# MGI-tech-bioinformatics/SuperPlus

Hardware: AMD Instinct MI355X
Metric: k-mers/s (DF createDict stage: trim + canonical k-mer count + solid filter + spectrum + adjacency) (higher is better)
Workload: dtype u64

## Files before the change

superplus_amd/csrc/dfk_kernels.h:

```cpp
#pragma once
#include <type_traits>
#include "dfk_device.h"
#include "dfk_fallback.h"
#include "dfk_scan_plan.h"

namespace dfk {

template <int K>
__global__ void __launch_bounds__(256)
k_trim(const uint8_t* __restrict__ pq, const uint64_t* __restrict__ pq_off, uint64_t pq_nbytes,
       const uint64_t* __restrict__ base_off, uint64_t packed_bytes, const uint32_t* __restrict__ read_len,
       uint64_t n_reads, uint32_t min_qual, uint32_t* __restrict__ good_len,
       unsigned long long* __restrict__ n_inst, unsigned int* __restrict__ bad,
       unsigned long long* __restrict__ sum_good)
{
    unsigned long long mine = 0, good = 0;
    bool any_bad = false;
    for (uint64_t r = (uint64_t)blockIdx.x * blockDim.x + threadIdx.x; r < n_reads; r += (uint64_t)gridDim.x * blockDim.x) {
        uint32_t gl = 0;
        uint64_t p = pq_off[r], end = pq_off[r + 1];
        uint32_t idx = 0, run = 0;
        const uint64_t b0 = base_off[r], b1 = base_off[r + 1];
        bool ok = p <= end && end <= pq_nbytes && b0 <= b1 && b1 <= packed_bytes && b1 - b0 >= ((uint64_t)read_len[r] + 3) / 4;
        if (!ok) end = p;
// ... 13 lines not shown
                uint64_t bit = 8 * (p + 1) + 9;
                const uint32_t fmask = (1u << nBits) - 1u;
                for (uint32_t left = nQs; left;) {
                    const uint64_t by = bit >> 3;
                    const uint32_t sh = (uint32_t)(bit & 7);
                    uint64_t w = 0;
                    if (by + 8 <= pq_nbytes) __builtin_memcpy(&w, pq + by, 8);
                    else for (uint32_t k = 0; k < 8 && by + k < pq_nbytes; ++k) w |= (uint64_t)pq[by + k] << (8 * k);
                    w >>= sh;
                    const uint32_t n = min(left, (64u - sh) / nBits);
                    for (uint32_t i = 0; i < n; ++i, w >>= nBits) {
                        const uint32_t q = minQ + ((uint32_t)w & fmask);
                        if (q < min_qual) run = 0;
                        else if (++run >= (uint32_t)K) gl = idx + 1;
                        ++idx;
                    }
                    bit += (uint64_t)n * nBits; left -= n;
                }
            }
            p += blk;
        }
        uint32_t rl = read_len[r];
        if (!ok || idx != rl) { any_bad = true; gl = 0; }
        if (gl > rl) gl = rl;
        good_len[r] = gl;
        good += gl;
        if (gl >= (uint32_t)K + 1) mine += gl - K + 1;
    }
    __shared__ unsigned long long sh[2][4];
    __shared__ unsigned int sh_bad;
    if (threadIdx.x == 0) sh_bad = 0;
    __syncthreads();
#pragma unroll
    for (int d = 32; d > 0; d >>= 1) { mine += __shfl_down(mine, d, 64); good += __shfl_down(good, d, 64); }
    if ((threadIdx.x & 63) == 0) { sh[0][threadIdx.x >> 6] = mine; sh[1][threadIdx.x >> 6] = good; }
    if (any_bad) atomicOr(&sh_bad, 1u);
    __syncthreads();
    if (threadIdx.x == 0) {
        unsigned long long a0 = sh[0][0] + sh[0][1] + sh[0][2] + sh[0][3], a1 = sh[1][0] + sh[1][1] + sh[1][2] + sh[1][3];
        if (a0) atomicAdd(n_inst, a0);
        if (a1) atomicAdd(sum_good, a1);
        if (sh_bad) atomicOr(bad, 1u);
    }
}

struct PartParams {
    uint32_t M;
    uint32_t W;
    uint32_t log2_nb;
    uint32_t log2_world;
    int64_t  read_id0;
    uint32_t sub_lo;
    uint32_t sub_n;
    uint32_t class_mask;
};

constexpr uint32_t SWEEP_CLASSES = 32;
__host__ __device__ inline uint32_t sweep_class_of(uint32_t local_bucket, uint32_t log2_local)
{ return log2_local > 5 ? local_bucket >> (log2_local - 5) : local_bucket; }
__host__ __device__ inline uint32_t sweep_class_mask(uint32_t sub_lo, uint32_t sub_n, uint32_t log2_local)
{
    if (sub_n == 0) return 0u;
    const uint32_t a = sweep_class_of(sub_lo, log2_local), b = sweep_class_of(sub_lo + sub_n - 1, log2_local);
    const uint32_t upto_b = b >= 31 ? 0xFFFFFFFFu : ((1u << (b + 1)) - 1u);
    return upto_b & ~((1u << a) - 1u);
}

constexpr uint32_t SUMMARY_OVERFLOW = 15;

__device__ __forceinline__ uint32_t pass_local(uint32_t bucket, const PartParams& pp)
{
    const uint32_t ls = pp.log2_nb - pp.log2_world;
    const uint32_t d = (bucket & ((1u << ls) - 1u)) - pp.sub_lo;
    return d < pp.sub_n ? (bucket >> ls) * pp.sub_n + d : 0xFFFFFFFFu;
}

__device__ __forceinline__ uint32_t bucket_of(uint32_t minhash, const PartParams& pp)
{
    const uint32_t b = (minhash * 0x9E3779B1u) >> (32 - pp.log2_nb);
    return ((b & ((1u << pp.log2_world) - 1u)) << (pp.log2_nb - pp.log2_world)) | (b >> pp.log2_world);
}
constexpr int PART_QCAP = 8;

template <int K>
__device__ __forceinline__ void emit_record(const uint32_t* __restrict__ words, uint64_t n_words, uint64_t bit0,
                                            uint32_t s0, uint32_t nk, uint32_t bucket, uint32_t gl, int32_t tag,
                                            uint64_t dst_index, uint4* __restrict__ records)
{
    const bool hp = s0 > 0;
    const bool hs = s0 + nk + (uint32_t)K <= gl;
    uint64_t bo = bit0 + 2ull * (hp ? s0 - 1 : 0);
    uint64_t wi = bo >> 5; uint32_t sh = (uint32_t)bo & 31u;
    uint32_t w[7];
#pragma unroll
    for (int i = 0; i < 7; ++i) w[i] = (wi + i < n_words) ? words[wi + i] : 0u;
    uint32_t o[6];
#pragma unroll
    for (int i = 0; i < 6; ++i) o[i] = alignbit(w[i + 1], w[i], sh);
    if (!hp) {
#pragma unroll
        for (int i = 5; i > 0; --i) o[i] = (o[i] << 2) | (o[i - 1] >> 30);
        o[0] <<= 2;
    }
    uint32_t nbits = 2u * (1u + nk + (uint32_t)K - 1u + (hs ? 1u : 0u));
#pragma unroll
    for (int i = 0; i < 6; ++i) {
        uint32_t lo = 32u * i;
        if (nbits <= lo) o[i] = 0;
        else if (nbits < lo + 32u) o[i] &= (1u << (nbits - lo)) - 1u;
    }
    uint4 a{rec_header(nk, hp, hs, bucket), (uint32_t)tag, o[0], o[1]};
    uint4 b{o[2], o[3], o[4], o[5]};
    records[2 * dst_index] = a;
    records[2 * dst_index + 1] = b;
}

__device__ __forceinline__ uint32_t class_bin(uint32_t bucket, const PartParams& pp)
{
    const uint32_t ls = pp.log2_nb - pp.log2_world;
    const uint32_t sub = bucket & ((1u << ls) - 1u);
    return (bucket >> ls) * PART_CLASSES + (ls > 6 ? sub >> (ls - 6) : sub);
}

template <int K, bool WRITE>
__device__ __forceinline__ void
partition_read(uint64_t r, uint32_t* smem, uint32_t* __restrict__ lh,
            const uint8_t* __restrict__ packed, uint64_t packed_bytes, const uint64_t* __restrict__ base_off,
            const uint32_t* __restrict__ good_len, const int32_t* __restrict__ bc, int64_t ign_bc_below,
            uint64_t n_reads, const PartParams& pp,
            unsigned long long* __restrict__ bucket_acc, unsigned long long* __restrict__ bucket_cur, uint64_t n_out,
            uint4* __restrict__ records, uint4* __restrict__ summaries, const uint32_t* __restrict__ read_list, uint64_t n_list,
            const uint64_t* __restrict__ slice_base, uint32_t* __restrict__ read_classes)
{
    auto place = [&](uint32_t b) -> uint64_t {
        if (!slice_base) { const uint64_t d = atomicAdd(&bucket_cur[b], 1ull); return d < n_out ? d : ~0ull; }
        const uint32_t owner = b / pp.sub_n;
        const uint64_t d = slice_base[owner] + atomicAdd(&bucket_cur[owner], 1ull);
        return d < slice_base[owner + 1] ? d : ~0ull;
    };
    uint32_t* arr = smem;
    uint32_t* queue = smem + pp.W * PART_THREADS;
    uint8_t* sidx = reinterpret_cast<uint8_t*>(smem + pp.W * PART_THREADS);
    uint32_t* ring = reinterpret_cast<uint32_t*>(sidx + pp.W * PART_THREADS);
    uint64_t sum_lo = 0, sum_hi = 0;
    const int tid = threadIdx.x;
    if (WRITE && read_list) { if (r >= n_list) return; r = read_list[r]; }
    const uint32_t M = pp.M, W = pp.W;
    const uint32_t gl = r < n_reads ? good_len[r] : 0;
    if (gl < (uint32_t)K + 1) {
        if (!WRITE && r < n_reads) { summaries[r] = uint4{0, 0, 0, 0}; if (read_classes) read_classes[r] = 0u; }
        return;
    }
    uint32_t Pi = 0, cur_rel = 0;
    uint32_t cmask = 0;
    const uint32_t log2_local = pp.log2_nb - pp.log2_world;

    const uint64_t byte0 = base_off[r];
    const uint32_t* words = reinterpret_cast<const uint32_t*>(packed);
    const uint64_t n_words = (packed_bytes + 3) >> 2;
    const uint64_t bit0 = byte0 * 8;
    int32_t tag = -1;
    if (bc && (int64_t)r + pp.read_id0 >= ign_bc_below) tag = bc[r];

    const uint32_t mmask = M == 16 ? 0xFFFFFFFFu : ((1u << (2 * M)) - 1u);
    const uint32_t rsh = 2 * (M - 1);
    uint32_t f = 0, rc = 0;
    uint32_t P = 0;
    uint32_t bi = 0;
    uint32_t cur_b = 0, cur_s0 = 0, cur_nk = 0;
    uint32_t qn = 0;

    uint64_t wi = bit0 >> 5;
    uint64_t filled_to = wi;
    auto fill = [&]() {
        uint32_t w[PART_RING];
#pragma unroll
        for (int k = 0; k < PART_RING; ++k) w[k] = filled_to + k < n_words ? words[filled_to + k] : 0u;
#pragma unroll
        for (int k = 0; k < PART_RING; ++k) ring[((filled_to + k) & (PART_RING - 1)) * PART_THREADS + tid] = w[k];
        filled_to += PART_RING;
    };
    uint32_t wbits, wnext = 0;
    if (!WRITE) { fill(); wbits = ring[(wi & (PART_RING - 1)) * PART_THREADS + tid]; }
    else { wbits = wi < n_words ? words[wi] : 0u; wnext = wi + 1 < n_words ? words[wi + 1] : 0u; }
    uint32_t wpos = (uint32_t)bit0 & 31u;
    uint32_t sfx_next = 0xFFFFFFFFu;

    auto close_run = [&]() {
        if (WRITE && cur_b == 0xFFFFFFFFu) return;
        if (!WRITE) {
            if (lh) { const uint32_t bin = class_bin(cur_b, pp); atomicAdd(&lh[bin], 1u); atomicAdd(&lh[(PART_CLASSES << pp.log2_world) + bin], cur_nk); }
            else atomicAdd(&bucket_acc[cur_b], (1ull << 32) | cur_nk);
            cmask |= 1u << sweep_class_of(cur_b & ((1u << log2_local) - 1u), log2_local);
            if (qn < (uint32_t)SUMMARY_RUNS) {
                const uint64_t fld = cur_nk | (cur_rel << 6);
                const uint32_t b = 8u + 12u * qn;
                if (b < 64u) { sum_lo |= fld << b; if (b > 52u) sum_hi |= fld >> (64u - b); }
// ... 365 lines not shown
    extern __shared__ uint32_t lh[];
    const uint32_t c = blockIdx.y;
    for (uint32_t i = threadIdx.x; i < n_sub; i += blockDim.x) lh[i] = 0;
    __syncthreads();
    const uint64_t n = min((uint64_t)fill[c], cap);
    const uint32_t* k = keys + c * cap;
    for (uint64_t t0 = (uint64_t)blockIdx.x * KEY_TILE; t0 < n; t0 += (uint64_t)gridDim.x * KEY_TILE) {
        const uint64_t t1 = min(n, t0 + KEY_TILE);
        uint4 v[KEY_VECS];
        key_tile_load(k, t0, t1, v);
        key_tile_each(t0, t1, v, [&](uint32_t key) { atomicAdd(&lh[key >> sh], 1u); });
    }
    __syncthreads();
    for (uint32_t i = threadIdx.x; i < n_sub; i += blockDim.x) if (lh[i]) atomicAdd(&sub_cnt[(uint64_t)c * n_sub + i], (unsigned long long)lh[i]);
}

__global__ void __launch_bounds__(1024)
k_keys_offsets(const unsigned long long* __restrict__ cnt, uint32_t n, unsigned long long* __restrict__ off, unsigned long long* __restrict__ cur)
{
    __shared__ unsigned long long part[1024];
    const uint32_t tid = threadIdx.x, per = (n + 1023) / 1024;
    const uint32_t lo = min(n, tid * per), hi = min(n, lo + per);
    unsigned long long s = 0;
    for (uint32_t i = lo; i < hi; ++i) s += cnt[i];
    part[tid] = s;
    __syncthreads();
    for (uint32_t d = 1; d < 1024; d <<= 1) {
        const unsigned long long v = tid >= d ? part[tid - d] : 0ull;
        __syncthreads();
        part[tid] += v;
        __syncthreads();
    }
    unsigned long long run = part[tid] - s;
    for (uint32_t i = lo; i < hi; ++i) { off[i] = run; cur[i] = run; run += cnt[i]; }
    if (tid == 1023) off[n] = part[1023];
}

__global__ void __launch_bounds__(256)
k_keys_partition(const uint32_t* __restrict__ keys, const unsigned long long* __restrict__ fill, uint64_t cap, uint32_t sh,
                 uint32_t n_sub, unsigned long long* __restrict__ cur, uint32_t* __restrict__ out)
{
    extern __shared__ unsigned long long lds64[];
    unsigned long long* base = lds64;
    uint32_t* lh = reinterpret_cast<uint32_t*>(lds64 + n_sub);
    const uint32_t c = blockIdx.y;
    const uint64_t n = min((uint64_t)fill[c], cap);
    const uint32_t* k = keys + c * cap;
    unsigned long long* cc = cur + (uint64_t)c * n_sub;
    for (uint64_t t0 = (uint64_t)blockIdx.x * KEY_TILE; t0 < n; t0 += (uint64_t)gridDim.x * KEY_TILE) {
        const uint64_t t1 = min(n, t0 + KEY_TILE);
        uint4 v[KEY_VECS];
        key_tile_load(k, t0, t1, v);
        for (uint32_t i = threadIdx.x; i < n_sub; i += blockDim.x) lh[i] = 0;
        __syncthreads();
        key_tile_each(t0, t1, v, [&](uint32_t key) { atomicAdd(&lh[key >> sh], 1u); });
        __syncthreads();
        for (uint32_t i = threadIdx.x; i < n_sub; i += blockDim.x) { if (lh[i]) base[i] = atomicAdd(&cc[i], (unsigned long long)lh[i]); lh[i] = 0; }
        __syncthreads();
        uint32_t sh2 = sh;
        asm volatile("" : "+s"(sh2));
        key_tile_each(t0, t1, v, [&](uint32_t key) { const uint32_t s = key >> sh2; out[base[s] + atomicAdd(&lh[s], 1u)] = key; });
        __syncthreads();
    }
}

__global__ void __launch_bounds__(1024)
k_keys_count(const uint32_t* __restrict__ part, const unsigned long long* __restrict__ off, uint32_t sb, unsigned long long* __restrict__ bucket_acc)
{
    __shared__ unsigned long long t[1u << KEY_SUB_BITS];
    const uint32_t s = blockIdx.x, nt = 1u << sb, m = nt - 1u;
    for (uint32_t i = threadIdx.x; i < nt; i += blockDim.x) t[i] = 0;
    __syncthreads();
    const uint64_t a = off[s], b = off[s + 1];
    for (uint64_t i = a + threadIdx.x; i < b; i += blockDim.x) {
        const uint32_t key = part[i];
        atomicAdd(&t[(key >> 6) & m], (1ull << 32) | (key & 63u));
    }
    __syncthreads();
    unsigned long long* dst = bucket_acc + ((uint64_t)s << sb);
    for (uint32_t i = threadIdx.x; i < nt; i += blockDim.x) if (t[i]) atomicAdd(&dst[i], t[i]);
}

constexpr int SLICE_READS = 16;
template <int K, bool EMIT, typename F>
__device__ __forceinline__ void for_each_run_in_pass(uint64_t r, const uint8_t* __restrict__ packed, uint64_t packed_bytes,
                                                     const uint64_t* __restrict__ base_off, const PartParams& pp,
                                                     const uint4* __restrict__ summaries, F&& f)
{
    const uint4 sm = summaries[r];
    const uint32_t n = sm.x & 15u;
    if (n == 0 || n == SUMMARY_OVERFLOW) return;
    const uint32_t* words = reinterpret_cast<const uint32_t*>(packed);
    const uint64_t n_words = (packed_bytes + 3) >> 2;
    const uint64_t bit0 = base_off[r] * 8;
    const uint32_t M = pp.M;
    const uint32_t mmask = M == 16 ? 0xFFFFFFFFu : ((1u << (2 * M)) - 1u);
    const uint64_t lo = (uint64_t)sm.x | ((uint64_t)sm.y << 32), hi = (uint64_t)sm.z | ((uint64_t)sm.w << 32);
    uint32_t s0 = 0;
#pragma unroll
    for (int i = 0; i < SUMMARY_RUNS; ++i) {
        if ((uint32_t)i < n) {
            constexpr int B0 = 8;
            const int b = B0 + 12 * i;
            const uint32_t fld = (uint32_t)(b + 12 <= 64 ? lo >> b : b >= 64 ? hi >> (b - 64) : (lo >> b) | (hi << (64 - b))) & 0xFFFu;
            const uint32_t nk = fld & 63u, rel = fld >> 6;
            const uint64_t bo = bit0 + 2ull * (s0 + rel);
            const uint64_t wi = bo >> 5;
            const uint32_t w0 = words[wi], w1 = wi + 1 < n_words ? words[wi + 1] : 0u;
            const uint32_t x = alignbit(w1, w0, (uint32_t)bo & 31u) & mmask;
            uint32_t y = __brev(x);
            y = ((y >> 1) & 0x55555555u) | ((y & 0x55555555u) << 1);
            const uint32_t fw = y >> (32 - 2 * M), rcv = ~x & mmask;
            const uint32_t bucket = bucket_of(mmer_hash(fw < rcv ? fw : rcv), pp);
            const uint32_t lb = pass_local(bucket, pp);
            if (lb != 0xFFFFFFFFu) f(s0, nk, lb, bucket >> (pp.log2_nb - pp.log2_world), bit0, (uint32_t)i + 1 == n);
            s0 += nk;
        }
    }
}

template <int K>
__global__ void __launch_bounds__(256)
k_scatter_slices(const uint8_t* __restrict__ packed, uint64_t packed_bytes, const uint64_t* __restrict__ base_off,
                 const uint32_t* __restrict__ good_len, const int32_t* __restrict__ bc, int64_t ign_bc_below,
                 uint64_t n_reads, PartParams pp, const uint4* __restrict__ summaries, const uint32_t* __restrict__ read_classes,
                 const uint64_t* __restrict__ slice_base,
                 unsigned long long* __restrict__ slice_fill,
                 uint4* __restrict__ records)
{
    __shared__ uint32_t cnt[256];
    __shared__ unsigned long long at[256];
    __shared__ uint16_t list[256 * SLICE_READS];
    __shared__ uint32_t n_list;
    const uint32_t world = 1u << pp.log2_world;
    const int lane = threadIdx.x & 63;
    const uint64_t r_block = (uint64_t)blockIdx.x * 256 * SLICE_READS;
    if (threadIdx.x < world) cnt[threadIdx.x] = 0;
    if (threadIdx.x == 0) n_list = 0;
    __syncthreads();
#pragma unroll
    for (int j = 0; j < SLICE_READS; ++j) {
        const uint32_t rel = 256u * j + threadIdx.x;
        const uint64_t r = r_block + rel;
        const bool hit = r < n_reads && (!read_classes || (read_classes[r] & pp.class_mask) != 0u);
        const unsigned long long mk = __ballot(hit);
        uint32_t w = 0;
        if (lane == 0 && mk) w = atomicAdd(&n_list, (uint32_t)__popcll(mk));
        w = __builtin_amdgcn_readfirstlane(w);
        if (hit) list[w + __popcll(mk & ((1ull << lane) - 1ull))] = (uint16_t)rel;
    }
    __syncthreads();
    const uint32_t n = n_list;
    for (uint32_t i = threadIdx.x; i < n; i += 256)
        for_each_run_in_pass<K, false>(r_block + list[i], packed, packed_bytes, base_off, pp, summaries,
                                       [&](uint32_t, uint32_t, uint32_t, uint32_t owner, uint64_t, bool) { atomicAdd(&cnt[owner], 1u); });
    __syncthreads();
    if (threadIdx.x < world) {
        const uint32_t m = cnt[threadIdx.x];
        at[threadIdx.x] = slice_base[threadIdx.x] + (m ? atomicAdd(&slice_fill[threadIdx.x], (unsigned long long)m) : 0ull);
        cnt[threadIdx.x] = 0;
    }
    __syncthreads();
    const uint32_t* words = reinterpret_cast<const uint32_t*>(packed);
    const uint64_t n_words = (packed_bytes + 3) >> 2;
    (void)good_len;
    for (uint32_t i = threadIdx.x; i < n; i += 256) {
        const uint64_t r = r_block + list[i];
        int32_t tag = -1;
        if (bc && (int64_t)r + pp.read_id0 >= ign_bc_below) tag = bc[r];
        for_each_run_in_pass<K, true>(r, packed, packed_bytes, base_off, pp, summaries,
            [&](uint32_t s0, uint32_t nk, uint32_t lb, uint32_t owner, uint64_t bit0, bool last) {
                const uint64_t dst = at[owner] + atomicAdd(&cnt[owner], 1u);
                if (dst < slice_base[owner + 1]) emit_record<K>(words, n_words, bit0, s0, nk, lb, last ? 0u : 0xFFFFFFFFu, tag, dst, records);
            });
    }
}

#ifndef DFK_SWEEP_READS
#define DFK_SWEEP_READS 8
#endif
template <int K> constexpr int sweep_reads() { return KTraits<K>::KW == 4 ? 2 : DFK_SWEEP_READS; }
template <int K>
__global__ void __launch_bounds__(256)
k_scatter_runs(const uint8_t* __restrict__ packed, uint64_t packed_bytes, const uint64_t* __restrict__ base_off,
               const uint32_t* __restrict__ good_len, const int32_t* __restrict__ bc, int64_t ign_bc_below,
               uint64_t n_reads, PartParams pp, const uint4* __restrict__ summaries, const uint32_t* __restrict__ read_classes,
               unsigned long long* __restrict__ bucket_cur, uint64_t n_out, uint4* __restrict__ records)
{
    constexpr int SWEEP_READS = sweep_reads<K>();
    __shared__ uint16_t list[256 * SWEEP_READS];
    __shared__ uint32_t n_list;
    (void)good_len;
    const int lane = threadIdx.x & 63;
    const uint64_t r_block = (uint64_t)blockIdx.x * 256 * SWEEP_READS;
    if (threadIdx.x == 0) n_list = 0;
    __syncthreads();
#pragma unroll
    for (int j = 0; j < SWEEP_READS; ++j) {
        const uint32_t rel = 256u * j + threadIdx.x;
        const uint64_t r = r_block + rel;
        const bool hit = r < n_reads && (read_classes[r] & pp.class_mask) != 0u;
        const unsigned long long mk = __ballot(hit);
        uint32_t at = 0;
        if (lane == 0 && mk) at = atomicAdd(&n_list, (uint32_t)__popcll(mk));
        at = __builtin_amdgcn_readfirstlane(at);
        if (hit) list[at + __popcll(mk & ((1ull << lane) - 1ull))] = (uint16_t)rel;
    }
    __syncthreads();
    const uint32_t n = n_list;
    const uint32_t* words = reinterpret_cast<const uint32_t*>(packed);
    const uint64_t n_words = (packed_bytes + 3) >> 2;
    for (uint32_t i = threadIdx.x; i < n; i += 256) {
        const uint64_t r = r_block + list[i];
        int32_t tag = -1;
        if (bc && (int64_t)r + pp.read_id0 >= ign_bc_below) tag = bc[r];
        for_each_run_in_pass<K, true>(r, packed, packed_bytes, base_off, pp, summaries,
            [&](uint32_t s0, uint32_t nk, uint32_t lb, uint32_t, uint64_t bit0, bool last) {
                const uint64_t dst = atomicAdd(&bucket_cur[lb], 1ull);
                if (dst < n_out) emit_record<K>(words, n_words, bit0, s0, nk, lb, last ? 0u : 0xFFFFFFFFu, tag, dst, records);
            });
    }
}



struct CountParams {
    uint32_t min_freq, min_bc;
    uint32_t n_items;
    uint32_t single;
    uint64_t seg_cap;
    uint32_t do_adj;
    uint32_t keep_pre;
};

struct CountGlobals {
    unsigned long long n_distinct;
    unsigned long long big_cursor;
    unsigned int next_item;
    unsigned int n_overflow;
    unsigned int solid_overflow;
    unsigned int n_split;
    unsigned long long n_boundary;
    unsigned long long part_cursor;
    unsigned int n_wg_idle;
    unsigned int pad_idle;
};

constexpr int COUNT_HIST_BINS = 256;
constexpr uint32_t COUNT_MAX_PROBE = 96;
constexpr uint32_t HIST_GLOBAL_BINS = 1u << 24;
constexpr uint32_t FLAG_SOLID = 0x80000000u;

template <int K> struct WaveStage {
    uint32_t rec[COUNT_CHUNK * 8 + 8];
    uint32_t starts[COUNT_CHUNK];
    uint32_t msk[64];
    uint32_t pc[64];
};

__device__ __forceinline__ uint32_t tld(const uint32_t* p)
{ return __hip_atomic_load(p, __ATOMIC_RELAXED, __HIP_MEMORY_SCOPE_AGENT); }
__device__ __forceinline__ void tst(uint32_t* p, uint32_t v)
{ __hip_atomic_store(p, v, __ATOMIC_RELAXED, __HIP_MEMORY_SCOPE_AGENT); }

struct Probe {
    uint32_t k0, k1, k2, k3, ctx, fp, step, slot;
    int32_t tag;
    bool active;
};

__device__ __forceinline__ Probe probe_begin(u128 c, uint32_t ctx, int32_t tag, uint32_t S, bool active)
{
    const uint32_t h = key_hash(c);
    return Probe{(uint32_t)c.lo, (uint32_t)(c.lo >> 32), (uint32_t)c.hi, (uint32_t)(c.hi >> 32), ctx, (h >> 24) | 1u,
                 ((h >> 11) | 1u) & (S - 1), h & (S - 1), tag, active};
}

#define DFK_COMPILER_FENCE() asm volatile("" ::: "memory")
#ifdef DFK_PHASE_TIMES
__device__ unsigned long long g_phase[16];
struct PhaseClock {
    unsigned long long t, acc[12];
    __device__ __forceinline__ void start() { t = __builtin_amdgcn_s_memtime(); for (int i = 0; i < 12; ++i) acc[i] = 0; }
    __device__ __forceinline__ void mark(int i) { const unsigned long long n = __builtin_amdgcn_s_memtime(); acc[i] += n - t; t = n; }
    __device__ __forceinline__ void flush(int lane) { if (lane == 0) for (int i = 0; i < 12; ++i) atomicAdd(&g_phase[i], acc[i]); }
};
#define PH(i) phase.mark(i)
#else
#define PH(i) do { } while (0)
#endif
__device__ unsigned int g_big_fail[4];

enum : uint32_t { PS_PROBING = 0, PS_FOUND = 1, PS_FAILED = 2, PS_IDLE = 3 };
constexpr uint32_t PROBE_COST = 1u << 12, PROBE_LIMIT = (COUNT_MAX_PROBE + 1) * PROBE_COST;

template <int KW, int NBC, bool LDS_TABLE>
__device__ __forceinline__ bool table_insert(uint32_t* __restrict__ keys, uint32_t* __restrict__ cnt,
                                             uint32_t* __restrict__ ctxs, uint32_t* __restrict__ bcw,
                                             uint32_t S, const Probe& A, uint32_t& n_claimed)
{
    uint32_t state = A.active ? PS_PROBING : PS_IDLE, slot = A.slot, seen = 0, cost = 0, waits = 0;
    while (__ballot(state == PS_PROBING) != 0ull) {
        if (state == PS_PROBING) {
            uint32_t e = 0, r0, r1, r2, r3 = A.k3;
            if (LDS_TABLE) {
                __hip_atomic_compare_exchange_strong(&cnt[slot], &e, CNT_LOCK, __ATOMIC_RELAXED, __ATOMIC_RELAXED,
                                                     __HIP_MEMORY_SCOPE_WORKGROUP);
                DFK_COMPILER_FENCE();
                r0 = tld(&keys[slot]); r1 = tld(&keys[S + slot]); r2 = tld(&keys[2 * S + slot]);
                if (KW == 4) r3 = tld(&keys[3 * S + slot]);
            } else {
                __hip_atomic_compare_exchange_strong(&cnt[slot], &e, CNT_LOCK, __ATOMIC_ACQUIRE, __ATOMIC_ACQUIRE,
                                                     __HIP_MEMORY_SCOPE_AGENT);
                r0 = tld(&keys[slot]); r1 = tld(&keys[S + slot]); r2 = tld(&keys[2 * S + slot]);
                if (KW == 4) r3 = tld(&keys[3 * S + slot]);
            }
            const bool won = e == 0u;
            if (won) {
                tst(&keys[slot], A.k0); tst(&keys[S + slot], A.k1); tst(&keys[2 * S + slot], A.k2);
                if (KW == 4) tst(&keys[3 * S + slot], A.k3);
                if (LDS_TABLE) {
                    DFK_COMPILER_FENCE();
                    __hip_atomic_store(&cnt[slot], A.fp << 24, __ATOMIC_RELAXED, __HIP_MEMORY_SCOPE_WORKGROUP);
                } else __hip_atomic_store(&cnt[slot], A.fp << 24, __ATOMIC_RELEASE, __HIP_MEMORY_SCOPE_AGENT);
            }
            const uint32_t locked = e == CNT_LOCK;
            const uint32_t match = ((e >> 24) == A.fp) & (r0 == A.k0) & (r1 == A.k1) & (r2 == A.k2) & (r3 == A.k3);
            const uint32_t fin = (uint32_t)won | match;
            n_claimed += (uint32_t)won;
            seen |= e & (0u - match);
            cost += PROBE_COST - (PROBE_COST - 1u) * locked;
            if (!LDS_TABLE) waits += locked;
            slot = (slot + (A.step & ((fin | locked) - 1u))) & (S - 1);
            state = fin | ((uint32_t)(cost >= PROBE_LIMIT) << 1);
        }
    }
    if (!LDS_TABLE && state == PS_FAILED && atomicCAS(&g_big_fail[0], 0u, 1u) == 0u) {
        g_big_fail[1] = (cost - waits) / PROBE_COST; g_big_fail[2] = waits; g_big_fail[3] = 31u - (uint32_t)__clz(S);
    }
    if (state == PS_FOUND) {
        if (LDS_TABLE) {
// ... 390 lines not shown
            PH(7);
        } else {
            for (uint32_t lo = 0; lo < S; lo += ADJ_TASKS / 8) {
                __syncthreads();
                if (tid == 0) tst(n_tasks, 0u);
                __syncthreads();
                for (uint32_t slot = lo + tid; slot < min(S, lo + ADJ_TASKS / 8); slot += nthreads) {
                    if (!(tld(&cnt[slot]) && (tld(&bcw[slot]) & FLAG_SOLID))) continue;
                    const uint32_t ctx = tld(&ctxs[slot]) & 0xFFu;
                    uint32_t pos = atomicAdd(n_tasks, __popc(ctx));
                    for (uint32_t bit = 0; bit < 8; ++bit) if (ctx & (1u << bit)) tasks[pos++] = slot | (bit << 28);
                }
                __syncthreads();
                const uint32_t n = __builtin_amdgcn_readfirstlane(tld(n_tasks));
                for (uint32_t t = tid; t < n; t += nthreads) resolve(tasks[t]);
            }
            sync();
        }
    }
    else sync();
    uint32_t boundary = 0;
    auto emit = [&](uint32_t slot, uint32_t c, uint32_t flags, unsigned long long idx) {
        const uint32_t count = c & CNT_MASK;
        const uint32_t cw = tld(&ctxs[slot]);
        const uint32_t pending = flags & 0xFFu & cw;
        boundary += pending != 0;
        if (idx < cp.seg_cap) {
            u128 v{(uint64_t)tld(&keys[slot]) | ((uint64_t)tld(&keys[S + slot]) << 32),
                   (uint64_t)tld(&keys[2 * S + slot]) | (KW == 4 ? ((uint64_t)tld(&keys[3 * S + slot]) << 32) : 0ull)};
            u128 kw = shl128(v, 128 - KTraits<K>::BITS);
            seg_out[2 * idx] = uint4{(uint32_t)kw.hi, (uint32_t)(kw.hi >> 32), (uint32_t)kw.lo, (uint32_t)(kw.lo >> 32)};
            seg_out[2 * idx + 1] = uint4{0xFFFFFFFFu, count | ((cw & 0xFFu) << 24), 0xFFFFFFFFu, pending | (cw & 0xFF00u)};
        } else atomicOr(seg_overflow, 1u);
        if (count < (uint32_t)COUNT_HIST_BINS) atomicAdd(&hist_lds[count], 1u);
        else atomicAdd(&hist_global[count], 1ull);
    };
    {
        const uint32_t ns = __builtin_amdgcn_readfirstlane(tld(n_solid));
        const uint32_t used = __builtin_amdgcn_readfirstlane(tld(&ctl[CTL_USED]));
        const unsigned long long cur = uniform64(tld(&ctl[CTL_OUT_LO]), tld(&ctl[CTL_OUT_HI]));
        const unsigned long long nxt = uniform64(tld(&ctl[CTL_NEXT_LO]), tld(&ctl[CTL_NEXT_HI]));
        for (uint32_t i = tid; i < ns; i += nthreads) {
            const uint32_t slot = solid_list[i];
            const uint32_t pos = used + i;
            emit(slot, tld(&cnt[slot]), tld(&bcw[slot]), pos < OUT_CHUNK ? cur + pos : nxt + (pos - OUT_CHUNK));
        }
        PH(8);
        __syncthreads();
        PH(9);
        if (tid == 0) {
            if (used + ns > OUT_CHUNK) { tst(&ctl[CTL_OUT_LO], (uint32_t)nxt); tst(&ctl[CTL_OUT_HI], (uint32_t)(nxt >> 32)); tst(&ctl[CTL_USED], used + ns - OUT_CHUNK); }
            else tst(&ctl[CTL_USED], used + ns);
            tst(n_solid, 0u);
        }
        uint4* z = reinterpret_cast<uint4*>(cnt);
        for (uint32_t i = tid; i < (3 + (NBC > 1 ? NBC - 1 : 0)) * S / 4; i += nthreads) z[i] = uint4{0, 0, 0, 0};
    }
    boundary = wave_sum(boundary);
    if (lane == 0 && boundary) atomicAdd(n_boundary, boundary);
    PH(10);
    return n_occ;
}


template <int K, int LOG2S, int NWAVES, int NBC, bool SUB>
__global__ void __launch_bounds__(NWAVES * 64)
k_count(const uint4* __restrict__ records, const ItemRange* __restrict__ items, const uint64_t* __restrict__ rec_base,
        CountParams cp, CountGlobals* __restrict__ g, uint4* __restrict__ out, WgOut* __restrict__ wg_out,
        unsigned long long* __restrict__ hist_global, ItemRange* __restrict__ overflow_items,
        const uint32_t* __restrict__ item_sub,
        unsigned int* __restrict__ resident)
{
    constexpr uint32_t S = 1u << LOG2S;
    constexpr int KW = KTraits<K>::KW;
    constexpr int NT = NWAVES * 64;
    extern __shared__ __align__(16) uint32_t smem[];
    uint32_t* keys = smem;
    uint32_t* cnt = keys + KW * S;
    uint32_t* ctxs = cnt + S;
    uint32_t* bcw = ctxs + S;
    constexpr uint32_t XW = NBC > 1 ? NBC - 1 : 0;
    uint32_t* hist = bcw + (1 + XW) * S;
    uint32_t* ctl = hist + COUNT_HIST_BINS;
    uint32_t* tasks = ctl + CTL_N;
    uint16_t* solid_list = reinterpret_cast<uint16_t*>(tasks + S / 2);
    WaveStage<K>* stages = reinterpret_cast<WaveStage<K>*>(tasks + S / 2 + S / 2);
    const int tid = threadIdx.x, lane = tid & 63, wave = tid >> 6;
    WaveStage<K>* st = stages + wave;
    uint4* seg_out = out;

    if (tid == 0 && resident) __hip_atomic_fetch_add(resident, 1u, __ATOMIC_RELAXED, __HIP_MEMORY_SCOPE_AGENT);
    for (int i = tid; i < COUNT_HIST_BINS; i += NT) hist[i] = 0;
    for (uint32_t i = tid; i < (3 + XW) * S; i += NT) cnt[i] = 0;
    if (tid == 0) {
        const WgOut w = wg_out[blockIdx.x];
        ctl[CTL_OUT_LO] = (uint32_t)w.chunk; ctl[CTL_OUT_HI] = (uint32_t)(w.chunk >> 32); ctl[CTL_USED] = w.used;
        ctl[CTL_NEXT_LO] = 0; ctl[CTL_NEXT_HI] = 0; ctl[CTL_DISTINCT] = 0; ctl[CTL_BOUNDARY] = 0;
        ctl[CTL_OVF] = 0; ctl[CTL_FILL] = 0; ctl[CTL_CHUNK] = 0; ctl[CTL_NTASK] = 0; ctl[CTL_NSOLID] = 0; ctl[CTL_SP] = 0;
        const uint32_t it0 = atomicAdd(&g->next_item, 1u);
        uint64_t b0 = 0, e0 = 0; ItemRange r0{0, 0}; uint32_t s0 = 0;
        if (it0 < cp.n_items) { r0 = items[it0]; b0 = rec_base[r0.b0]; e0 = rec_base[r0.b1]; if (SUB) s0 = item_sub[it0]; }
        ctl[CTL_ITEM] = it0; ctl[CTL_RB_LO] = (uint32_t)b0; ctl[CTL_RB_HI] = (uint32_t)(b0 >> 32);
        ctl[CTL_RE_LO] = (uint32_t)e0; ctl[CTL_RE_HI] = (uint32_t)(e0 >> 32);
        ctl[CTL_B0] = r0.b0; ctl[CTL_B1] = r0.b1; ctl[CTL_SUB] = s0;
    }
#ifdef DFK_PHASE_TIMES
    PhaseClock phase; phase.start();
#endif
    uint32_t items_done = 0;
    for (;;) {
        PH(0);
        __syncthreads();
        PH(1);
        const uint32_t item = __builtin_amdgcn_readfirstlane(ctl[CTL_ITEM]);
        if (item >= cp.n_items) break;
        ++items_done;
        const uint64_t rb = uniform64(ctl[CTL_RB_LO], ctl[CTL_RB_HI]);
        const uint64_t re = uniform64(ctl[CTL_RE_LO], ctl[CTL_RE_HI]);
        const uint32_t sub = __builtin_amdgcn_readfirstlane(ctl[CTL_SUB]);
        uint32_t nx = 0xFFFFFFFFu; uint64_t nb = 0, ne = 0; ItemRange nr{0, 0}; uint32_t nsub = 0;
        if (tid == 0 && ctl[CTL_SP] == 0) {
            nx = atomicAdd(&g->next_item, 1u);
            if (nx < cp.n_items) { nr = items[nx]; nb = rec_base[nr.b0]; ne = rec_base[nr.b1]; if (SUB) nsub = item_sub[nx]; }
        }
        const uint32_t n_rec = (uint32_t)(re - rb);
        const uint32_t share = (n_rec + NWAVES - 1) / NWAVES;
        const uint32_t wv = __builtin_amdgcn_readfirstlane((uint32_t)wave);
        const uint32_t w_lo = min(n_rec, wv * share), w_hi = min(n_rec, w_lo + share);
        if (!SUB && cp.single) {
            for (uint32_t at = w_lo; at < w_hi; at += 64) {
                if (__builtin_amdgcn_readfirstlane(tld(&ctl[CTL_OVF]))) break;
                const uint32_t r = at + (uint32_t)lane;
                uint4 a{0, 0, 0, 0}, b{0, 0, 0, 0};
                if (r < w_hi) { a = records[2 * (rb + r)]; b = records[2 * (rb + r) + 1]; }
                const InstRegs in{a.x, a.y, a.z, a.w, b.x, b.y, b.z, 0u};
                const Probe A = make_probe<K>(in, S, (a.x & 63u) != 0u);
                uint32_t claimed = 0;
                const bool ok = table_insert<KW, NBC, true>(keys, cnt, ctxs, bcw, S, A, claimed);
                claimed = wave_sum(claimed);
                if (lane == 0 && claimed) atomicAdd(&ctl[CTL_FILL], claimed);
                if (!ok) atomicOr(&ctl[CTL_OVF], 1u);
                if (lane == 0 && tld(&ctl[CTL_FILL]) > (S / 4) * 3) tst(&ctl[CTL_OVF], 1u);
            }
        } else
        for (uint32_t at = w_lo; at < w_hi; at += COUNT_CHUNK) {
            if (__builtin_amdgcn_readfirstlane(tld(&ctl[CTL_OVF]))) break;
            wave_count_chunk<K, NBC, true, SUB>(records, rb + at, rb + w_hi, st, lane, keys, cnt, ctxs, bcw, S,
                                             &ctl[CTL_FILL], &ctl[CTL_OVF], sub);
            if (lane == 0 && tld(&ctl[CTL_FILL]) > (S / 4) * 3) tst(&ctl[CTL_OVF], 1u);
        }
        PH(2);
        __syncthreads();
        PH(3);
        if (__builtin_amdgcn_readfirstlane(ctl[CTL_OVF])) {
            if (tid == 0) {
                const uint32_t b0 = ctl[CTL_B0], b1 = ctl[CTL_B1];
                uint32_t sp = ctl[CTL_SP];
                if (b1 - b0 > 1 && sp + 3 <= (uint32_t)CTL_STACK_CAP) {
                    if (nx < cp.n_items) { ctl[CTL_STACK + 3 * sp] = nr.b0; ctl[CTL_STACK + 3 * sp + 1] = nr.b1; ctl[CTL_STACK + 3 * sp + 2] = nsub; ++sp; nx = 0xFFFFFFFFu; }
                    const uint32_t mid = b0 + (b1 - b0) / 2;
                    ctl[CTL_STACK + 3 * sp] = mid; ctl[CTL_STACK + 3 * sp + 1] = b1; ctl[CTL_STACK + 3 * sp + 2] = 0u; ++sp;
                    ctl[CTL_STACK + 3 * sp] = b0; ctl[CTL_STACK + 3 * sp + 1] = mid; ctl[CTL_STACK + 3 * sp + 2] = 0u; ++sp;
                    ctl[CTL_SP] = sp;
                    atomicAdd(&g->n_split, 1u);
                } else overflow_items[atomicAdd(&g->n_overflow, 1u)] = ItemRange{b0, SUB ? (0x80000000u | ctl[CTL_SUB]) : b1};
            }
            for (uint32_t i = tid; i < (3 + XW) * S; i += NT) cnt[i] = 0;
            __syncthreads();
        } else {
            uint32_t occ = table_finish<K, NBC, S / 2>(keys, cnt, ctxs, bcw, S, cp, seg_out, ctl, &g->part_cursor,
                                                         &g->solid_overflow, hist, hist_global, tasks, &ctl[CTL_NTASK],
                                                         &ctl[CTL_BOUNDARY], solid_list, &ctl[CTL_NSOLID], tid, NT
#ifdef DFK_PHASE_TIMES
                                                         , phase
#endif
                                                         );
            occ = wave_sum(occ);
            if (lane == 0 && occ) atomicAdd(&ctl[CTL_DISTINCT], occ);
        }
        if (tid == 0) {
            const uint32_t sp = ctl[CTL_SP];
            uint32_t n0 = nr.b0, n1 = nr.b1;
            if (sp) {
                n0 = ctl[CTL_STACK + 3 * (sp - 1)]; n1 = ctl[CTL_STACK + 3 * (sp - 1) + 1]; nsub = ctl[CTL_STACK + 3 * (sp - 1) + 2];
                ctl[CTL_SP] = sp - 1;
                nx = 0; nb = rec_base[n0]; ne = rec_base[n1];
            }
            ctl[CTL_ITEM] = nx; ctl[CTL_RB_LO] = (uint32_t)nb; ctl[CTL_RB_HI] = (uint32_t)(nb >> 32);
            ctl[CTL_RE_LO] = (uint32_t)ne; ctl[CTL_RE_HI] = (uint32_t)(ne >> 32);
            ctl[CTL_B0] = n0; ctl[CTL_B1] = n1; ctl[CTL_SUB] = nsub;
            ctl[CTL_OVF] = 0; ctl[CTL_FILL] = 0; ctl[CTL_CHUNK] = 0; ctl[CTL_NTASK] = 0;
        }
    }
    __syncthreads();
#ifdef DFK_PHASE_TIMES
    PH(11); phase.flush(lane);
#endif
    for (int i = tid; i < COUNT_HIST_BINS; i += NT) if (hist[i]) atomicAdd(&hist_global[i], (unsigned long long)hist[i]);
    if (tid == 0) {
        wg_out[blockIdx.x] = WgOut{(unsigned long long)ctl[CTL_OUT_LO] | ((unsigned long long)ctl[CTL_OUT_HI] << 32), ctl[CTL_USED], 0u};
        if (ctl[CTL_DISTINCT]) atomicAdd(&g->n_distinct, (unsigned long long)ctl[CTL_DISTINCT]);
        if (ctl[CTL_BOUNDARY]) atomicAdd(&g->n_boundary, (unsigned long long)ctl[CTL_BOUNDARY]);
        if (!items_done) atomicAdd(&g->n_wg_idle, 1u);
    }
}

__global__ void __launch_bounds__(64)
k_gate(const unsigned int* __restrict__ ctr, unsigned int target, unsigned long long max_ticks, unsigned int* __restrict__ timed_out)
{
    if (threadIdx.x != 0) return;
    const unsigned long long t0 = wall_clock64();
    while ((int)(__hip_atomic_load(ctr, __ATOMIC_RELAXED, __HIP_MEMORY_SCOPE_AGENT) - target) < 0) {
        if (wall_clock64() - t0 > max_ticks) { __hip_atomic_fetch_add(timed_out, 1u, __ATOMIC_RELAXED, __HIP_MEMORY_SCOPE_AGENT); break; }
        __builtin_amdgcn_s_sleep(64);
    }
}

template <int K, int LOG2S, int NWAVES, int NBC>
constexpr size_t count_lds_bytes()
{
    return sizeof(uint32_t) * ((size_t)(KTraits<K>::KW + 3 + (NBC > 1 ? NBC - 1 : 0)) * (1u << LOG2S) + COUNT_HIST_BINS + CTL_N + (1u << LOG2S) / 2 + (1u << LOG2S) / 2) + sizeof(WaveStage<K>) * NWAVES;
}

template <int K, int NWAVES, int NBC>
__global__ void __launch_bounds__(NWAVES * 64)
k_big_insert(const uint4* __restrict__ records, const BigItem* __restrict__ items, const uint64_t* __restrict__ rec_base,
             const uint64_t* __restrict__ chunk_pre, uint32_t n_items, uint32_t* __restrict__ tab_pool,
             unsigned long long* __restrict__ ticket, uint32_t* __restrict__ failed)
{
    constexpr int KW = KTraits<K>::KW;
    __shared__ WaveStage<K> stages[NWAVES];
    __shared__ uint32_t fill, ovf;
    const int lane = threadIdx.x & 63, wave = threadIdx.x >> 6;
    if (threadIdx.x == 0) { fill = 0; ovf = 0; }
    __syncthreads();
    const uint64_t n_chunks = chunk_pre[n_items];
    for (uint32_t guard = 0; guard < 0x7FFFFFFFu; ++guard) {
        unsigned long long t0 = 0;
        if (lane == 0) t0 = atomicAdd(ticket, (unsigned long long)BIG_TICKET_CHUNKS);
        const uint64_t first = uniform64((uint64_t)t0);
        if (first >= n_chunks) break;
        for (int k = 0; k < BIG_TICKET_CHUNKS; ++k) {
            const uint64_t t = first + k;
            if (t >= n_chunks) break;
            const uint32_t it = big_find(chunk_pre, n_items, t);
            const BigItem I = items[it];
            const uint32_t S = 1u << I.log2s;
            uint32_t* keys = tab_pool + I.tab_off;
            uint32_t* cnt = keys + (size_t)KW * S;
            const uint64_t rb = rec_base[I.b0] + (t - chunk_pre[it]) * COUNT_CHUNK;
            wave_count_chunk<K, NBC, false>(records, rb, rec_base[I.b1], &stages[wave], lane, keys, cnt, cnt + S, cnt + 3 * (size_t)S, S, &fill, &ovf);
        }
    }
    __syncthreads();
    if (threadIdx.x == 0 && ovf) atomicOr(failed, 1u);
}

template <int K> struct BigView {
    uint32_t* keys; uint32_t* cnt; uint32_t* ctxs; uint32_t* wide; uint32_t* bcw; uint32_t S, slot;
    __device__ __forceinline__ uint32_t count() const { const uint32_t c = tld(&wide[slot]); return c < CNT_MASK ? c : CNT_MASK; }
};
template <int K>
__device__ __forceinline__ BigView<K> big_view(const BigItem* __restrict__ items, const uint64_t* __restrict__ slot_pre, uint32_t n_items,
                                               uint32_t* __restrict__ tab_pool, uint64_t x)
{
    const uint32_t it = big_find(slot_pre, n_items, x);
    const BigItem I = items[it];
    const uint32_t S = 1u << I.log2s;
    uint32_t* keys = tab_pool + I.tab_off;
    uint32_t* cnt = keys + (size_t)KTraits<K>::KW * S;
    return BigView<K>{keys, cnt, cnt + S, cnt + 2 * (size_t)S, cnt + 3 * (size_t)S, S, (uint32_t)(x - slot_pre[it])};
}

template <int K, int NBC>
__global__ void __launch_bounds__(256)
k_big_flags(const BigItem* __restrict__ items, const uint64_t* __restrict__ slot_pre, uint32_t n_items, uint32_t* __restrict__ tab_pool,
            CountParams cp, CountGlobals* __restrict__ g)
{
    const uint64_t total = slot_pre[n_items];
    uint32_t occ = 0;
    for (uint64_t x = (uint64_t)blockIdx.x * 256 + threadIdx.x; x < total; x += (uint64_t)gridDim.x * 256) {
        const BigView<K> v = big_view<K>(items, slot_pre, n_items, tab_pool, x);
        const uint32_t c = tld(&v.cnt[v.slot]);
        if (!c) continue;
        ++occ;
        const bool solid = v.count() >= cp.min_freq && bc_pass<(NBC > 0)>(NBC > 0 ? tld(&v.bcw[v.slot]) : 0u, cp.min_bc);
        if (solid && cp.do_adj && cp.keep_pre) { const uint32_t ctx = tld(&v.ctxs[v.slot]) & 0xFFu; tst(&v.ctxs[v.slot], ctx | (ctx << 8)); }
        tst(&v.bcw[v.slot], solid ? FLAG_SOLID : 0u);
    }
#pragma unroll
    for (int d = 32; d > 0; d >>= 1) occ += __shfl_down(occ, d, 64);
    if ((threadIdx.x & 63) == 0 && occ) atomicAdd(&g->n_distinct, (unsigned long long)occ);
}

template <int K>
__global__ void __launch_bounds__(256)
k_big_resolve(const BigItem* __restrict__ items, const uint64_t* __restrict__ slot_pre, uint32_t n_items, uint32_t* __restrict__ tab_pool)
{
    constexpr int KW = KTraits<K>::KW;
    const uint64_t total = slot_pre[n_items];
    const u128 m = KTraits<K>::mask();
    for (uint64_t x = (uint64_t)blockIdx.x * 256 + threadIdx.x; x < total; x += (uint64_t)gridDim.x * 256) {
        const BigView<K> v = big_view<K>(items, slot_pre, n_items, tab_pool, x);
        if (!tld(&v.cnt[v.slot]) || !(tld(&v.bcw[v.slot]) & FLAG_SOLID)) continue;
// ... 667 lines not shown
```

Before: 65.53 billion.

## Restructure scatter kernel into batched sweep with prefetch and alias count LDS lists

```diff
diff --git a/superplus_amd/csrc/dfk_kernels.h b/superplus_amd/csrc/dfk_kernels.h
--- a/superplus_amd/csrc/dfk_kernels.h
+++ b/superplus_amd/csrc/dfk_kernels.h
@@ -119,37 +119,50 @@
 }
 constexpr int PART_QCAP = 8;
 
+__device__ __forceinline__ void record_window_load(const uint32_t* __restrict__ words, uint64_t n_words, uint64_t bit0,
+                                                   uint32_t s0, uint32_t (&w)[7])
+{
+    const uint64_t wi = (bit0 + 2ull * (s0 > 0 ? s0 - 1 : 0)) >> 5;
+#pragma unroll
+    for (int i = 0; i < 7; ++i) w[i] = (wi + i < n_words) ? words[wi + i] : 0u;
+}
+
+template <int K>
+__device__ __forceinline__ void record_write(const uint32_t (&w)[7], uint64_t bit0, uint32_t s0, uint32_t nk, uint32_t bucket,
+                                             uint32_t gl, int32_t tag, uint64_t dst_index, uint4* __restrict__ records)
+{
+    const bool hp = s0 > 0;
+    const bool hs = s0 + nk + (uint32_t)K <= gl;
+    const uint32_t sh = (uint32_t)(bit0 + 2ull * (hp ? s0 - 1 : 0)) & 31u;
+    uint32_t o[6];
+#pragma unroll
+    for (int i = 0; i < 6; ++i) o[i] = alignbit(w[i + 1], w[i], sh);
+    if (!hp) {
+#pragma unroll
+        for (int i = 5; i > 0; --i) o[i] = (o[i] << 2) | (o[i - 1] >> 30);
+        o[0] <<= 2;
+    }
+    uint32_t nbits = 2u * (1u + nk + (uint32_t)K - 1u + (hs ? 1u : 0u));
+#pragma unroll
+    for (int i = 0; i < 6; ++i) {
+        uint32_t lo = 32u * i;
+        if (nbits <= lo) o[i] = 0;
+        else if (nbits < lo + 32u) o[i] &= (1u << (nbits - lo)) - 1u;
+    }
+    uint4 a{rec_header(nk, hp, hs, bucket), (uint32_t)tag, o[0], o[1]};
+    uint4 b{o[2], o[3], o[4], o[5]};
+    records[2 * dst_index] = a;
+    records[2 * dst_index + 1] = b;
+}
+
 template <int K>
 __device__ __forceinline__ void emit_record(const uint32_t* __restrict__ words, uint64_t n_words, uint64_t bit0,
                                             uint32_t s0, uint32_t nk, uint32_t bucket, uint32_t gl, int32_t tag,
                                             uint64_t dst_index, uint4* __restrict__ records)
 {
-    const bool hp = s0 > 0;
-    const bool hs = s0 + nk + (uint32_t)K <= gl;
-    uint64_t bo = bit0 + 2ull * (hp ? s0 - 1 : 0);
-    uint64_t wi = bo >> 5; uint32_t sh = (uint32_t)bo & 31u;
     uint32_t w[7];
-#pragma unroll
-    for (int i = 0; i < 7; ++i) w[i] = (wi + i < n_words) ? words[wi + i] : 0u;
-    uint32_t o[6];
-#pragma unroll
-    for (int i = 0; i < 6; ++i) o[i] = alignbit(w[i + 1], w[i], sh);
-    if (!hp) {
-#pragma unroll
-        for (int i = 5; i > 0; --i) o[i] = (o[i] << 2) | (o[i - 1] >> 30);
-        o[0] <<= 2;
-    }
-    uint32_t nbits = 2u * (1u + nk + (uint32_t)K - 1u + (hs ? 1u : 0u));
-#pragma unroll
-    for (int i = 0; i < 6; ++i) {
-        uint32_t lo = 32u * i;
-        if (nbits <= lo) o[i] = 0;
-        else if (nbits < lo + 32u) o[i] &= (1u << (nbits - lo)) - 1u;
-    }
-    uint4 a{rec_header(nk, hp, hs, bucket), (uint32_t)tag, o[0], o[1]};
-    uint4 b{o[2], o[3], o[4], o[5]};
-    records[2 * dst_index] = a;
-    records[2 * dst_index + 1] = b;
+    record_window_load(words, n_words, bit0, s0, w);
+    record_write<K>(w, bit0, s0, nk, bucket, gl, tag, dst_index, records);
 }
 
 __device__ __forceinline__ uint32_t class_bin(uint32_t bucket, const PartParams& pp)
@@ -681,6 +694,11 @@
 }
 
 constexpr int SLICE_READS = 16;
+__device__ __forceinline__ uint32_t summary_field(uint64_t lo, uint64_t hi, int i)
+{
+    const int b = 8 + 12 * i;
+    return (uint32_t)(b + 12 <= 64 ? lo >> b : b >= 64 ? hi >> (b - 64) : (lo >> b) | (hi << (64 - b))) & 0xFFFu;
+}
 template <int K, bool EMIT, typename F>
 __device__ __forceinline__ void for_each_run_in_pass(uint64_t r, const uint8_t* __restrict__ packed, uint64_t packed_bytes,
                                                      const uint64_t* __restrict__ base_off, const PartParams& pp,
@@ -699,9 +717,7 @@
 #pragma unroll
     for (int i = 0; i < SUMMARY_RUNS; ++i) {
         if ((uint32_t)i < n) {
-            constexpr int B0 = 8;
-            const int b = B0 + 12 * i;
-            const uint32_t fld = (uint32_t)(b + 12 <= 64 ? lo >> b : b >= 64 ? hi >> (b - 64) : (lo >> b) | (hi << (64 - b))) & 0xFFFu;
+            const uint32_t fld = summary_field(lo, hi, i);
             const uint32_t nk = fld & 63u, rel = fld >> 6;
             const uint64_t bo = bit0 + 2ull * (s0 + rel);
             const uint64_t wi = bo >> 5;
@@ -775,12 +791,96 @@
     }
 }
 
+constexpr int SWEEP_HITS = 2;
+constexpr uint32_t SWEEP_NONE = 0xFFFFFFFFu;
+struct SweepRead {
+    uint4 sm; uint64_t byte0;
+    __device__ __forceinline__ uint32_t n() const { const uint32_t c = sm.x & 15u; return c == SUMMARY_OVERFLOW ? 0u : c; }
+    __device__ __forceinline__ uint32_t sub() const { return ((uint32_t)byte0 & 3u) * 8u; }
+    __device__ __forceinline__ const uint32_t* rw(const uint32_t* __restrict__ words) const { return words + (byte0 >> 2); }
+};
+struct __attribute__((aligned(4))) SweepPair { uint32_t a, b; };
+struct SweepHits { uint32_t lb[SWEEP_HITS], runs; };
+
+__device__ __forceinline__ SweepRead sweep_read(uint64_t r, const uint64_t* __restrict__ base_off, const uint4* __restrict__ summaries)
+{
+    return SweepRead{summaries[r], base_off[r]};
+}
+
+constexpr int SWEEP_BATCH = SUMMARY_RUNS / 2;
+static_assert(2 * SWEEP_BATCH == SUMMARY_RUNS, "two batches cover a summary");
+
+template <int I0>
+__device__ __forceinline__ void sweep_min_words(const SweepRead& R, uint32_t n, const uint32_t* __restrict__ words, uint32_t s0,
+                                                uint32_t (&w)[SWEEP_BATCH][2])
+{
+    const uint64_t lo = (uint64_t)R.sm.x | ((uint64_t)R.sm.y << 32), hi = (uint64_t)R.sm.z | ((uint64_t)R.sm.w << 32);
+    const uint32_t* rw = R.rw(words);
+    const uint32_t sub = R.sub();
+#pragma unroll
+    for (int i = I0; i < I0 + SWEEP_BATCH; ++i) {
+        if ((uint32_t)i < n) {
+            const uint32_t fld = summary_field(lo, hi, i);
+            const SweepPair v = *reinterpret_cast<const SweepPair*>(rw + ((sub + 2u * (s0 + (fld >> 6))) >> 5));
+            w[i - I0][0] = v.a; w[i - I0][1] = v.b;
+            s0 += fld & 63u;
+        }
+    }
+}
+
+template <int I0>
+__device__ __forceinline__ void sweep_pick(const SweepRead& R, uint32_t n, const uint32_t (&w)[SWEEP_BATCH][2], const PartParams& pp,
+                                           uint32_t& s0, uint32_t& found, SweepHits& H)
+{
+    const uint64_t lo = (uint64_t)R.sm.x | ((uint64_t)R.sm.y << 32), hi = (uint64_t)R.sm.z | ((uint64_t)R.sm.w << 32);
+    const uint32_t M = pp.M;
+    const uint32_t mmask = M == 16 ? 0xFFFFFFFFu : ((1u << (2 * M)) - 1u);
+    const uint32_t sub = R.sub();
+#pragma unroll
+    for (int i = I0; i < I0 + SWEEP_BATCH; ++i) {
+        if ((uint32_t)i < n) {
+            const uint32_t fld = summary_field(lo, hi, i);
+            const uint32_t sh = (sub + 2u * (s0 + (fld >> 6))) & 31u;
+            const uint32_t x = alignbit(w[i - I0][1], w[i - I0][0], sh) & mmask;
+            uint32_t y = __brev(x);
+            y = ((y >> 1) & 0x55555555u) | ((y & 0x55555555u) << 1);
+            const uint32_t fw = y >> (32 - 2 * M), rcv = ~x & mmask;
+            const uint32_t lb = pass_local(bucket_of(mmer_hash(fw < rcv ? fw : rcv), pp), pp);
+            if (lb != SWEEP_NONE) {
+#pragma unroll
+                for (int g = 0; g < SWEEP_HITS; ++g) if (found == (uint32_t)g) { H.lb[g] = lb; H.runs |= (uint32_t)i << (4 * g); }
+                ++found;
+            }
+            s0 += fld & 63u;
+        }
+    }
+}
+
+__device__ __forceinline__ void sweep_window_load(const SweepRead& R, const uint32_t* __restrict__ words, uint32_t s0, uint32_t (&w)[7])
+{
+    const uint32_t* p = R.rw(words) + ((R.sub() + 2u * (s0 > 0 ? s0 - 1 : 0)) >> 5);
+#pragma unroll
+    for (int i = 0; i < 7; ++i) w[i] = p[i];
+}
+
+__device__ __forceinline__ void sweep_run(const SweepRead& R, uint32_t run, uint32_t& s0, uint32_t& nk)
+{
+    const uint64_t lo = (uint64_t)R.sm.x | ((uint64_t)R.sm.y << 32), hi = (uint64_t)R.sm.z | ((uint64_t)R.sm.w << 32);
+    s0 = 0; nk = 0;
+#pragma unroll
+    for (int i = 0; i < SUMMARY_RUNS; ++i) {
+        const uint32_t k = summary_field(lo, hi, i) & 63u;
+        if ((uint32_t)i < run) s0 += k;
+        if ((uint32_t)i == run) nk = k;
+    }
+}
+
 #ifndef DFK_SWEEP_READS
 #define DFK_SWEEP_READS 8
 #endif
 template <int K> constexpr int sweep_reads() { return KTraits<K>::KW == 4 ? 2 : DFK_SWEEP_READS; }
 template <int K>
-__global__ void __launch_bounds__(256)
+__global__ void __launch_bounds__(256, 8)
 k_scatter_runs(const uint8_t* __restrict__ packed, uint64_t packed_bytes, const uint64_t* __restrict__ base_off,
                const uint32_t* __restrict__ good_len, const int32_t* __restrict__ bc, int64_t ign_bc_below,
                uint64_t n_reads, PartParams pp, const uint4* __restrict__ summaries, const uint32_t* __restrict__ read_classes,
@@ -809,15 +909,73 @@
     const uint32_t n = n_list;
     const uint32_t* words = reinterpret_cast<const uint32_t*>(packed);
     const uint64_t n_words = (packed_bytes + 3) >> 2;
-    for (uint32_t i = threadIdx.x; i < n; i += 256) {
-        const uint64_t r = r_block + list[i];
+    const uint64_t r_end = r_block + 256ull * SWEEP_READS < n_reads ? r_block + 256ull * SWEEP_READS : n_reads;
+    if (base_off[r_end] + 32 > packed_bytes) {
+        for (uint32_t i = threadIdx.x; i < n; i += 256) {
+            const uint64_t r = r_block + list[i];
+            int32_t tag = -1;
+            if (bc && (int64_t)r + pp.read_id0 >= ign_bc_below) tag = bc[r];
+            for_each_run_in_pass<K, true>(r, packed, packed_bytes, base_off, pp, summaries,
+                [&](uint32_t s0, uint32_t nk, uint32_t lb, uint32_t, uint64_t bit0, bool last) {
+                    const uint64_t dst = atomicAdd(&bucket_cur[lb], 1ull);
+                    if (dst < n_out) emit_record<K>(words, n_words, bit0, s0, nk, lb, last ? 0u : 0xFFFFFFFFu, tag, dst, records);
+                });
+        }
+        return;
+    }
+    uint32_t i = threadIdx.x;
+    SweepRead R{};
+    if (i < n) R = sweep_read(r_block + list[i], base_off, summaries);
+    while (i < n) {
+        const uint32_t n_runs = R.n();
+        SweepHits H;
+#pragma unroll
+        for (int g = 0; g < SWEEP_HITS; ++g) H.lb[g] = SWEEP_NONE;
+        H.runs = 0u;
+        uint32_t before = 0, found = 0;
+        uint32_t w[SWEEP_BATCH][2];
+        sweep_min_words<0>(R, n_runs, words, before, w);
+        const SweepRead N = sweep_read(r_block + list[i + 256 < n ? i + 256 : i], base_off, summaries);
+        sweep_pick<0>(R, n_runs, w, pp, before, found, H);
+        if (__ballot(n_runs > (uint32_t)SWEEP_BATCH) != 0ull) {
+            sweep_min_words<SWEEP_BATCH>(R, n_runs, words, before, w);
+            sweep_pick<SWEEP_BATCH>(R, n_runs, w, pp, before, found, H);
+        }
+        uint32_t meta[SWEEP_HITS];
+#pragma unroll
+        for (int g = 0; g < SWEEP_HITS; ++g) {
+            const uint32_t run = (H.runs >> (4 * g)) & 15u;
+            uint32_t s0, nk;
+            sweep_run(R, run, s0, nk);
+            meta[g] = s0 | (nk << 16) | (run + 1u == n_runs ? 1u << 22 : 0u);
+        }
+        if (found > (uint32_t)SWEEP_HITS) meta[0] |= 1u << 23;
+        unsigned long long d[SWEEP_HITS];
+#pragma unroll
+        for (int g = 0; g < SWEEP_HITS; ++g) { d[g] = ~0ull; if (H.lb[g] != SWEEP_NONE) d[g] = atomicAdd(&bucket_cur[H.lb[g]], 1ull); }
         int32_t tag = -1;
-        if (bc && (int64_t)r + pp.read_id0 >= ign_bc_below) tag = bc[r];
-        for_each_run_in_pass<K, true>(r, packed, packed_bytes, base_off, pp, summaries,
-            [&](uint32_t s0, uint32_t nk, uint32_t lb, uint32_t, uint64_t bit0, bool last) {
-                const uint64_t dst = atomicAdd(&bucket_cur[lb], 1ull);
-                if (dst < n_out) emit_record<K>(words, n_words, bit0, s0, nk, lb, last ? 0u : 0xFFFFFFFFu, tag, dst, records);
-            });
+        if (H.lb[0] != SWEEP_NONE) {
+            const uint64_t r = r_block + list[i];
+            if (bc && (int64_t)r + pp.read_id0 >= ign_bc_below) tag = bc[r];
+        }
+#pragma unroll
+        for (int g = 0; g < SWEEP_HITS; ++g) {
+            if (H.lb[g] == SWEEP_NONE) continue;
+            uint32_t pw[7];
+            sweep_window_load(R, words, meta[g] & 0xFFFFu, pw);
+            if (d[g] < n_out) record_write<K>(pw, R.sub(), meta[g] & 0xFFFFu, (meta[g] >> 16) & 63u, H.lb[g], ((meta[g] >> 22) & 1u) ? 0u : 0xFFFFFFFFu, tag, d[g], records);
+        }
+        if (meta[0] >> 23) {
+            uint32_t seen = 0;
+            for_each_run_in_pass<K, true>(r_block + list[i], packed, packed_bytes, base_off, pp, summaries,
+                [&](uint32_t s0, uint32_t nk, uint32_t lb, uint32_t, uint64_t bit0, bool last) {
+                    if (seen++ < (uint32_t)SWEEP_HITS) return;
+                    const uint64_t dst = atomicAdd(&bucket_cur[lb], 1ull);
+                    if (dst < n_out) emit_record<K>(words, n_words, bit0, s0, nk, lb, last ? 0u : 0xFFFFFFFFu, tag, dst, records);
+                });
+        }
+        R = N;
+        i += 256;
     }
 }
 
@@ -856,6 +1014,7 @@
     uint32_t msk[64];
     uint32_t pc[64];
 };
+template <int LOG2S> constexpr size_t count_finish_bytes() { return sizeof(uint32_t) * ((1u << LOG2S) / 2) + sizeof(uint16_t) * (1u << LOG2S); }
 
 __device__ __forceinline__ uint32_t tld(const uint32_t* p)
 { return __hip_atomic_load(p, __ATOMIC_RELAXED, __HIP_MEMORY_SCOPE_AGENT); }
@@ -1412,9 +1571,11 @@
     constexpr uint32_t XW = NBC > 1 ? NBC - 1 : 0;
     uint32_t* hist = bcw + (1 + XW) * S;
     uint32_t* ctl = hist + COUNT_HIST_BINS;
+    static_assert((CTL_N % 4) == 0 && (S / 2) % 4 == 0 && sizeof(WaveStage<K>) % 16 == 0, "the staging areas and the lists stay 16-byte aligned");
+    static_assert(count_finish_bytes<LOG2S>() <= sizeof(WaveStage<K>) * NWAVES, "the finish lists fit the staging areas of this many waves");
     uint32_t* tasks = ctl + CTL_N;
     uint16_t* solid_list = reinterpret_cast<uint16_t*>(tasks + S / 2);
-    WaveStage<K>* stages = reinterpret_cast<WaveStage<K>*>(tasks + S / 2 + S / 2);
+    WaveStage<K>* stages = reinterpret_cast<WaveStage<K>*>(ctl + CTL_N);
     const int tid = threadIdx.x, lane = tid & 63, wave = tid >> 6;
     WaveStage<K>* st = stages + wave;
     uint4* seg_out = out;
@@ -1549,7 +1710,8 @@
 template <int K, int LOG2S, int NWAVES, int NBC>
 constexpr size_t count_lds_bytes()
 {
-    return sizeof(uint32_t) * ((size_t)(KTraits<K>::KW + 3 + (NBC > 1 ? NBC - 1 : 0)) * (1u << LOG2S) + COUNT_HIST_BINS + CTL_N + (1u << LOG2S) / 2 + (1u << LOG2S) / 2) + sizeof(WaveStage<K>) * NWAVES;
+    const size_t stage = sizeof(WaveStage<K>) * NWAVES, lists = count_finish_bytes<LOG2S>();
+    return sizeof(uint32_t) * ((size_t)(KTraits<K>::KW + 3 + (NBC > 1 ? NBC - 1 : 0)) * (1u << LOG2S) + COUNT_HIST_BINS + CTL_N) + (stage > lists ? stage : lists);
 }
 
 template <int K, int NWAVES, int NBC>
```

Result: no change. 66.10 billion, median of 6 (+0.9%).
